# tum-vision/povar

Measured on AMD Instinct MI355X. Metric: power-series iterations/s (solve_pOSE terms per second), higher is better.
Workload: dtype f64

## Files before the change

### povar_amd/csrc/ck_layout.hpp

```cpp
#pragma once

#include <climits>
#include <cmath>
#include <cstring>

#include "lpl_layout.hpp"

namespace povar {

#ifndef POVAR_CK_HMAX_BUILD
#define POVAR_CK_HMAX_BUILD 16
#endif
constexpr int CK_HMAX = POVAR_CK_HMAX_BUILD;
constexpr int CK_LDS_BYTES = 160 * 1024;
constexpr int CK_FLAG_DUP = 1;
constexpr int CK_FLAG_COLD = 2;
constexpr uint32_t CK_NONE = 0xffffu;

constexpr double CK_UV_SCALE = 1e6, CK_UV_INV = 1e-6;
inline double ck_unpack_uv_host(int32_t k) {
  const double kd = (double)k;
  const double q0 = kd * CK_UV_INV;
  const double r = std::fma(-q0, CK_UV_SCALE, kd);
  return std::fma(r, CK_UV_INV, q0);
// ... 389 lines not shown
  K.n_part_rec = first[n_cams];
  K.part_range.assign(n_cams, make_int2(0, 0));
  for (int r0 = 0; r0 < n_cams; ++r0) K.part_range[cam_of_rank[r0]] = make_int2(first[r0], first[r0 + 1]);
  K.slot_rec.assign(L.wg_cams.size(), 0);
  {
    std::vector<int> next(first.begin(), first.end() - 1);
    for (int w = 0; w < grid; ++w)
      for (size_t a = 0; a < acc_rank_of[w].size(); ++a) K.slot_rec[(size_t)L.wg_cam_off[w] + a] = next[acc_rank_of[w][a]]++;
    std::vector<int> cold_rec((size_t)n_cold_chunks);
    for (int w = 0; w < grid; ++w)
      for (size_t i = 0; i < out[w].cold_rank.size(); ++i) cold_rec[(size_t)cold0_of[w] + i] = next[out[w].cold_rank[i]]++;
    K.uv.assign((size_t)(K.rows + CK_HMAX) * WAVE, make_double2(0, 0));
    K.src.assign((size_t)(K.rows + CK_HMAX) * WAVE, -1);
    if (shape.cold_q) K.cpos.assign((size_t)(K.rows + CK_HMAX) * WAVE, -1);
    K.li.assign((size_t)(K.li_rows + CK_HMAX) * WAVE, CK_NONE | (CK_NONE << 16));
    K.lane_cam.resize(K.tile.size() * WAVE);
    K.lane_acc.resize(K.tile.size() * WAVE);
    K.lane_seg.resize(K.tile.size() * WAVE);
    lpl_parallel(grid, n_threads, [&](int w) {
      const WgOut& o = out[w];
      std::copy(o.uv.begin(), o.uv.end(), K.uv.begin() + row0_of[w] * WAVE);
      std::copy(o.src.begin(), o.src.end(), K.src.begin() + row0_of[w] * WAVE);
      if (shape.cold_q) std::copy(o.cpos.begin(), o.cpos.end(), K.cpos.begin() + row0_of[w] * WAVE);
      std::copy(o.li.begin(), o.li.end(), K.li.begin() + li0_of[w] * WAVE);
      std::copy(o.lane_cam.begin(), o.lane_cam.end(), K.lane_cam.begin() + (size_t)tile0_of[w] * WAVE);
      std::copy(o.lane_seg.begin(), o.lane_seg.end(), K.lane_seg.begin() + (size_t)tile0_of[w] * WAVE);
      for (size_t i = 0; i < o.lane_acc.size(); ++i) {
        const int a = o.lane_acc[i];
        K.lane_acc[(size_t)tile0_of[w] * WAVE + i] = a >= 0 ? a : shape.cold_q ? -1 : ~cold_rec[(size_t)cold0_of[w] + (size_t)(~a)];
      }
    });
  }
  K.n_uv = K.uv.size();
  {
    const char* e = std::getenv("POVAR_CK_PACK");
    if (shape.need_uv && shape.slot_bytes == 48 && pack_uv && !(e && e[0] == '0')) ck_pack_uv(K, n_threads);
  }
  K.tick.assign(K.tile.size() * WAVE, 0);
  lpl_parallel(grid, n_threads, [&](int w) {
    std::vector<int> next((size_t)std::max(1, L.wg_cam_off[w + 1] - L.wg_cam_off[w]), 0);
    for (int b = 0; b < nb; ++b) {
      const int tb0 = K.bt_off[(size_t)w * nb + b], tb1 = K.bt_off[(size_t)w * nb + b + 1];
      for (int q0 = tb0; q0 < tb1; q0 += n_waves)
        for (int t = std::min(q0 + n_waves, tb1) - 1; t >= q0; --t)
          for (int lane = 0; lane < WAVE; ++lane) {
            const size_t i = (size_t)t * WAVE + lane;
            if (K.lane_cam[i] >= 0 && K.lane_acc[i] >= 0 && lane == ((K.lane_seg[i] >> 8) & 255))
              K.tick[i] = (uint16_t)next[K.lane_acc[i]]++;
          }
    }
  });
}

}
```

### povar_amd/csrc/povar_create.hip

```cpp
#include "povar_ctx.hpp"

std::mutex g_capture_mu;

int hot_acc_cap(int n_cams) {
  int cap = HOT_ACC_MAX;
  if (const char* e = std::getenv("POVAR_HOT_ACC")) cap = std::max(1, std::min(HOT_ACC_MAX, std::atoi(e)));
  return std::min(n_cams, cap);
}

struct Layout {
  std::vector<double2> uv, cm_uv;
  std::vector<int> cam, lm, meta, hot_cams, cam_hot, cc_slot, cc_lm, cc_item_off, cc_cam_item_off, long_lm, long_first, long_cnt, cm_slot, cm_lm, item_off,
      item_cam, cam_item_off, slot_of_obs, cold_pos;
  std::vector<int> c2_lm, c2_pos;
  std::vector<int2> c2_range;
  int n_bins = 0;
};

struct LayoutTmp {
  std::vector<int> seg_first, seg_last, rank;
  std::vector<char> is_long;
  std::vector<int64_t> cnt;
};

// ... 132 lines not shown
      L.c2_range.resize(n_cams);
      for (int c = 0; c < n_cams; ++c) {
        const int first = (int)L.c2_lm.size();
        const bool acc = rank[c] > 0 && rank[c] <= n_acc;
        if (!acc)
          for (int64_t p = cnt[c]; p < cnt[c + 1]; ++p) {
            L.c2_pos[L.cm_slot[p]] = (int)L.c2_lm.size();
            L.c2_lm.push_back(L.cm_lm[p]);
          }
        L.c2_range[c] = make_int2(first, (int)L.c2_lm.size());
      }
    }
  }
}

int ck_max_cams() {
  if (const char* e = std::getenv("POVAR_CK_MAX_CAMS")) return std::max(0, std::atoi(e));
  return 65535;
}

bool ck_upload(povar_ctx* c, povar_ctx::CkDev& D, const CkLayout& K, bool locked, size_t* bytes, bool need_uv) {
  bool ok = true;
  const bool usable = K.n_uv * sizeof(double2) < (1ull << 32) && c->n_cams <= ck_max_cams();
  D.ready = false;
  if (!usable) return true;
  auto guarded = [&](auto&& fn) {
    if (locked) {
      std::lock_guard<std::mutex> lk(g_capture_mu);
      fn();
    } else {
      fn();
    }
  };
  auto up = [&](auto& buf, const auto& v) {
    if (!ok) return;
    guarded([&] { ok = buf.alloc(std::max<size_t>(v.size(), 1), bytes) == hipSuccess; });
    const size_t piece = ((size_t)8 << 20) / sizeof(v[0]);
    for (size_t at = 0; ok && at < v.size() && !(locked && c->placer_cancel.load()); at += piece)
      guarded([&] {
        ok = hipMemcpy(buf.p + at, v.data() + at, std::min(piece, v.size() - at) * sizeof(v[0]), hipMemcpyHostToDevice) == hipSuccess;
      });
  };
  std::vector<int2> meta(K.lane_cam.size());
  for (size_t i = 0; i < meta.size(); ++i) {
    const int sg = K.lane_seg[i];
    meta[i] = make_int2(K.lane_cam[i] < 0 ? -1 : (K.lane_cam[i] | ((sg & 63) << 16) | (((sg >> 8) & 63) << 22)), K.lane_acc[i]);
  }
  D.packed = need_uv && K.packed;
  if (D.packed) up(D.uvp, K.uvp);
  else if (need_uv) up(D.uv, K.uv);
  up(D.li, K.li); up(D.src, K.src); up(D.tile, K.tile); up(D.lane_meta, meta);
  up(D.bt_off, K.bt_off); up(D.slot_rec, K.slot_rec); up(D.part_range, K.part_range);
  if (c->det_ck) { up(D.lcnt, K.lcnt_log2); up(D.tick, K.tick); }
  D.cold_q = K.cold_q;
  if (K.cold_q) up(D.cpos, K.cpos);
  if (ok) guarded([&] { ok = D.part.alloc((size_t)std::max(K.n_part_rec, 1) * 12, bytes) == hipSuccess; });
  if (ok && c->opt.robust_norm && !need_uv)
    guarded([&] { ok = D.w.alloc(std::max<size_t>(K.src.size(), 1), bytes) == hipSuccess; });
  D.nb = K.nb; D.slots = K.slots; D.n_part_rec = K.n_part_rec; D.max_acc = K.max_acc; D.max_tiles_bt = K.max_tiles_bt;
  D.stride = K.stride; D.n_capped_obs = K.n_capped_obs;
  D.rows = K.rows; D.li_rows = K.li_rows; D.n_chunks = K.n_chunks; D.n_cold_chunks = K.n_cold_chunks;
  D.w_lin_id = -1;
  D.ready = ok && !(locked && c->placer_cancel.load());
  if (!ok) D.release();
  return ok;
}

int res_upload(povar_ctx* c, const ResLayout& R) {
  povar_ctx::ResDev& D = c->res;
  int rc = 0;
  if ((rc = upload(D.lane_cam, R.lane_cam, c)) || (rc = upload(D.lane_seg, R.lane_seg, c)) ||
      (rc = upload(D.uv, R.uv, c)) || (rc = upload(D.lslot, R.lslot, c)) || (rc = upload(D.oslot, R.oslot, c)) ||
      (rc = upload(D.wave_h, R.wave_h, c)) || (rc = upload(D.lm_off, R.lm_off, c)) || (rc = upload(D.lm_id, R.lm_id, c)) ||
      (rc = upload(D.cam_off, R.cam_off, c)) || (rc = upload(D.cam_id, R.cam_id, c)) || (rc = upload(D.cam_zi, R.cam_zi, c)) ||
      (rc = upload(D.own_off, R.own_off, c)) || (rc = upload(D.own_cam, R.own_cam, c)) || (rc = upload(D.own_zi, R.own_zi, c)) ||
      (rc = upload(D.own_q, R.own_q, c)) || (rc = upload(D.oq_off, R.oq_off, c)) || (rc = upload(D.oq_rec, R.oq_rec, c)))
    return rc;
  const size_t n_part = (size_t)std::max(R.n_rec, 1) * 12, n_z = (size_t)c->n_cams * 12, n_nrm = (size_t)RES_MAX_WG * 2 * 2;
  if (n_part * sizeof(uint4) >= (1ull << 32)) return fail(-1, "resident series: partial records exceed a buffer descriptor");
  HIP_TRY(D.part.alloc(n_part, &c->bytes));
  HIP_TRY(D.zbuf.alloc(n_z, &c->bytes));
  HIP_TRY(D.nrm.alloc(n_nrm, &c->bytes));
  HIP_TRY(D.launch.alloc(4, &c->bytes));
  HIP_TRY(hipMemset(D.part.p, 0, n_part * sizeof(uint4)));
  HIP_TRY(hipMemset(D.zbuf.p, 0, n_z * sizeof(uint4)));
  HIP_TRY(hipMemset(D.nrm.p, 0, n_nrm * sizeof(uint4)));
  const unsigned one[4] = {1u, 0u, 0u, 0u};
  HIP_TRY(hipMemcpy(D.launch.p, one, sizeof(one), hipMemcpyHostToDevice));
  D.W = R.W; D.NW = R.NW; D.H = R.H; D.R = R.R; D.LS = R.LS; D.n_rec = R.n_rec; D.max_lm = R.max_lm; D.max_cam = R.max_cam;
  D.max_oq = R.max_oq; D.max_own = R.max_own; D.max_chunks = R.max_chunks; D.order = R.order; D.lds_bytes = R.lds_bytes;
  D.ready = true;
  return 0;
}

void res_build_for(int n_cams, int n_lms, const int32_t* lm_off, const int32_t* cam_idx, const double* obs,
                   const std::vector<int>& rank1, const std::vector<int>& slot_of_obs, int wgs, ResLayout& R) {
  build_res(n_cams, n_lms, lm_off, cam_idx, obs, rank1, slot_of_obs, wgs, 16, 1, 1, 2, 1, R);
  if (R.fits) return;
  build_res(n_cams, n_lms, lm_off, cam_idx, obs, rank1, slot_of_obs, wgs, 8, 2, 1, 4, 2, R);
}

int swap_in_placed_rows(povar_ctx* c, bool wait) {
  if (c->placement != 2) return 0;
  if (!wait && c->placer_state.load(std::memory_order_acquire) < 2) return 0;
  if (c->placer.joinable()) c->placer.join();
  if (c->placer_state.load(std::memory_order_acquire) != 2) {
// ... 780 lines not shown
```

### povar_amd/csrc/povar_ctx.hpp

```cpp
#pragma once
#include "../../include/povar_hip.h"

#include <hip/hip_runtime.h>
#include <rccl/rccl.h>

#include <algorithm>
#include <chrono>
#include <cmath>
#include <cstdio>
#include <cstdlib>
#include <cstring>
#include <memory>
#include <mutex>
#include <numeric>
#include <string>
#include <atomic>
#include <thread>
#include <vector>

#include "povar_kernels.hpp"
#include "povar_kernels_joint.hpp"
#include "povar_kernels_sc.hpp"
#include "povar_kernels_chol.hpp"
#include "lpl_layout.hpp"
// ... 57 lines not shown
  int64_t n_cold = 0;
  int n_cold_items = 0;
  povar_options opt{};
  hipStream_t stream = nullptr;
  size_t bytes = 0;
  int64_t lin_id = 0, views_lin_id = -1, aux_lin_id = -1;
  int64_t prep_id = 0, aux_prep_id = 0, prep_lin_id = -1;
  char* pin = nullptr;
  size_t pin_bytes = 0;

  std::vector<int> slot_of_obs;
  std::vector<int> lm_off;

  DevBuf<double2> uv, cm_uv, tiles;
  DevBuf<int2> cc_cam_range;
  DevBuf<int> cold_pos;
  DevBuf<int> c2_lm, c2_pos;
  DevBuf<int2> c2_range;
  DevBuf<double> c2_h;
  int64_t n_cold2 = 0;
  bool long_in_kernel = false;
  DevBuf<double2> v2_uv;
  DevBuf<int> v2_lm_of;
  DevBuf<int> v2_cw, v2_cpos, v2_lm_pos, v2_of_slot, v2_seg, v2_wg_tile_off, v2_wg_cam_off, v2_wg_cams, v2_wg_slot_rec, c3_lm;
  DevBuf<int2> v2_part_range, c3_range;
  DevBuf<int> c3_src, pl_c3_src;
  bool q_rows = false;
  DevBuf<double> c3_h, v2_part;
  int64_t n_cold3 = 0;
  int v2_max_slots = 0, v2_n_global = 0, v2_n_tail = 0, v2_strategy = 0;
  DevBuf<int4> v2_tile;
  DevBuf<double> v2_w, v2_lmrec;
  int64_t v2_rows = 0;
  std::thread placer;
  std::atomic<int> placer_state{0};
  std::atomic<bool> placer_cancel{false};
  DevBuf<double2> pl_uv;
  DevBuf<int> pl_cw, pl_cpos, pl_lm_pos, pl_lm_of, pl_of_slot;
  size_t pl_bytes = 0;
  int placement = 0;
  double placement_ms = 0;
  bool use_lpl = true;
  bool lpl_forced = false;
  bool use_lpl_prepare = true;
  struct CkDev {
    DevBuf<double2> uv;
    DevBuf<int2> uvp;
    bool packed = false;
    DevBuf<int> cpos;
    bool cold_q = false;
    DevBuf<uint32_t> li;
    DevBuf<int> src, bt_off, slot_rec;
    DevBuf<int2> lane_meta;
    DevBuf<int4> tile;
    DevBuf<int2> part_range;
    DevBuf<double> part, w;
    DevBuf<uint8_t> lcnt;
    DevBuf<uint16_t> tick;
    int nb = 0, slots = 0, n_part_rec = 0, max_acc = 0, max_tiles_bt = 0;
    int stride = 0;
    int64_t n_capped_obs = 0;
    int64_t rows = 0, li_rows = 0, n_chunks = 0, n_cold_chunks = 0;
    double build_ms = 0;
    int64_t w_lin_id = -1;
    bool ready = false;
    void release() {
      cpos.release(); cold_q = false;
      uv.release(); uvp.release(); li.release(); src.release(); lane_meta.release(); bt_off.release();
      slot_rec.release(); tile.release(); part_range.release(); part.release(); w.release();
      packed = false;
      lcnt.release(); tick.release();
      ready = false;
    }
  } ck, pl_ck,
    ckh, pl_ckh;
  struct ResDev {
    DevBuf<int> lane_cam, lane_seg, lslot, oslot, wave_h, lm_off, lm_id, cam_off, cam_id, cam_zi, own_off, own_cam, own_zi, oq_off, oq_rec;
    DevBuf<double2> uv;
    DevBuf<int2> own_q;
    DevBuf<uint4> part, zbuf, nrm;
    DevBuf<unsigned> launch;
    int W = 0, NW = 0, H = 0, R = 1, LS = 1, n_rec = 0, max_lm = 0, max_cam = 0, max_oq = 0, max_own = 0, max_chunks = 0, order = 0;
    size_t lds_bytes = 0;
    double build_ms = 0;
    bool ready = false;
    void release() {
      lane_cam.release(); lane_seg.release(); lslot.release(); oslot.release(); wave_h.release();
      lm_off.release(); lm_id.release(); cam_off.release(); cam_id.release(); cam_zi.release(); own_off.release(); own_cam.release();
      own_zi.release(); oq_off.release(); oq_rec.release();
      uv.release(); own_q.release(); part.release(); zbuf.release(); nrm.release(); launch.release();
      ready = false;
    }
  } res;
  int res_mode = -1;
  bool res_tuned = false, res_choice = false, res_failed = false;
  float res_tune_us[2] = {0, 0};
  bool res_check = false;
  int res_last_m = 0;
  double res_last_tol[2] = {0, 0};
  unsigned res_spin_limit = 1u << 18;
  bool deterministic = false;
  bool det_ck = false;
  bool det_check = false;
  bool fp32_terms = false;
  bool fp32_hold = false;
  int32_t fp32_last = 0;
  DevBuf<float2> ck32_uv;
  DevBuf<float> ck32_lmrec;
  DevBuf<float> ck32_pimg;
  DevBuf<int2> ck_zero_range;
  int ck_variant = 0;
  int ckh_variant = 0;
  bool ckh_tuned = false;
  float ckh_tune_us[2] = {0, 0};
  bool ck_auto = true;
  bool ck_tuned = false;
  bool ck_fresh[2] = {false, false};
  float ck_tune_us[2] = {0, 0};
  DevBuf<double4> q4c;
  DevBuf<int> lm_slot0, lm_cnt_dev;
  bool k1_qr = true;
// ... 211 lines not shown
```

### povar_amd/csrc/povar_kernels_ck.hpp

```cpp
#pragma once

#include "povar_kernels.hpp"

namespace povar {

constexpr int CK_ROWS = 16;

struct CkP {
  const double2* uv;
  const uint32_t* li;
  const double* w;
  const int4* tile;
  const int2* lane_meta;
  const int* bt_off;
  const int* slot_rec;
  int nb, slots;
  unsigned uv_bytes, li_bytes;
  const uint8_t* lcnt;
  const uint16_t* tick;
  int max_acc;
  int uv_packed;
  const int* cpos;
  double4* q4c;
};
__device__ inline double ck_unpack_uv(unsigned k) {
  const double kd = (double)(int)k;
  const double q0 = kd * 1e-6;
  const double r = __builtin_fma(-q0, 1e6, kd);
  return __builtin_fma(r, 1e-6, q0);
}
typedef unsigned __attribute__((ext_vector_type(4))) ck_u4;
constexpr int CK_ACC_STRIDE = 13;
__host__ __device__ inline size_t ck_lds_bytes_dev(int slots, int n_acc, int ng) { return 16 + (size_t)ng * slots * 48 + (size_t)n_acc * CK_ACC_STRIDE * 8 + 64; }

__device__ inline void ck_barrier() { asm volatile("s_waitcnt lgkmcnt(0)\n\ts_barrier" ::: "memory"); }

__device__ inline void ck_group_barrier(int* cnt, int& gen, int group_waves, int lane) {
  asm volatile("s_waitcnt lgkmcnt(0)" ::: "memory");
  gen += group_waves;
  if (lane == 0) __hip_atomic_fetch_add(cnt, 1, __ATOMIC_RELAXED, __HIP_MEMORY_SCOPE_WORKGROUP);
  while (__hip_atomic_load(cnt, __ATOMIC_RELAXED, __HIP_MEMORY_SCOPE_WORKGROUP) < gen) __builtin_amdgcn_s_sleep(2);
  asm volatile("" ::: "memory");
}

__host__ __device__ inline int ck_rank(int x) { return x < 0 ? -1 : (x & 0xffff); }
__host__ __device__ inline int ck_seg(int x) { return ((x >> 16) & 63) | (((x >> 22) & 63) << 8); }

__device__ inline void ck_forward_math(const LplObs& o, const double* zz, const double* P3, double hx, double hy, double hz,
                                       double* red) {
  const double d0 = hx * zz[0] + hy * zz[1] + hz * zz[2] + zz[3];
  const double d1 = hx * zz[4] + hy * zz[5] + hz * zz[6] + zz[7];
  const double d2 = hx * zz[8] + hy * zz[9] + hz * zz[10] + zz[11];
  const double a0 = o.w * (d0 - o.cu * d2);
  const double a1 = o.w * (d1 - o.cv * d2);
  const double a2 = o.w * (o.cuv * d2 - o.cu * d0 - o.cv * d1);
  red[0] = P3[0] * a0 + P3[3] * a1 + P3[6] * a2;
  red[1] = P3[1] * a0 + P3[4] * a1 + P3[7] * a2;
  red[2] = P3[2] * a0 + P3[5] * a1 + P3[8] * a2;
}

__device__ inline double ck_huber_w(const Dp& d, const double* P3, double hx, double hy, double hz, double2 uv) {
  const double p0 = P3[0] * hx + P3[1] * hy + P3[2] * hz + P3[9];
  const double p1 = P3[3] * hx + P3[4] * hy + P3[5] * hz + P3[10];
  const double p2 = P3[6] * hx + P3[7] * hy + P3[8] * hz + P3[11];
  const double a = p0 - uv.x * p2, b = p1 - uv.y * p2, c = p0 - uv.x, e = p1 - uv.y;
  const double r2 = d.sb * d.sb * (a * a + b * b) + d.sa * d.sa * (c * c + e * e);
  const double t = d.huber;
  double y = __builtin_amdgcn_rsq(r2);
  const double hr = 0.5 * r2;
  y = y * __builtin_fma(-hr * y, y, 1.5);
  y = y * __builtin_fma(-hr * y, y, 1.5);
  return r2 < t * t ? 1.0 : t * y;
}

__device__ inline void ck_obs_forward(const Dp& d, double2 uv, double w, const double* zz, const double* P3, double hx, double hy,
                                      double hz, double* lu, int S, uint32_t s) {
  LplObs o;
  o.set(d, uv, w);
  double red[3];
  ck_forward_math(o, zz, P3, hx, hy, hz, red);
  __hip_atomic_fetch_add(lu + s, red[0], __ATOMIC_RELAXED, __HIP_MEMORY_SCOPE_WORKGROUP);
  __hip_atomic_fetch_add(lu + s + 1, red[1], __ATOMIC_RELAXED, __HIP_MEMORY_SCOPE_WORKGROUP);
  __hip_atomic_fetch_add(lu + s + 2, red[2], __ATOMIC_RELAXED, __HIP_MEMORY_SCOPE_WORKGROUP);
}
__device__ inline void ck_obs_backward(const Dp& d, double2 uv, double w, const double* P3, double hx, double hy, double hz,
                                       const double* g, double* y) {
  LplObs o;
  o.set(d, uv, w);
  double q[3];
  lpl_backward(o, P3, g, q);
#pragma unroll
  for (int m = 0; m < 3; ++m) {
    y[4 * m] += hx * q[m];
    y[4 * m + 1] += hy * q[m];
    y[4 * m + 2] += hz * q[m];
    y[4 * m + 3] += q[m];
  }
}

struct CkRows {
  __amdgpu_buffer_rsrc_t uv, li, w;
};
__device__ inline CkRows ck_rows(const CkP& k) {
  CkRows R;
  R.uv = __builtin_amdgcn_make_buffer_rsrc(const_cast<double2*>(k.uv), 0, k.uv_bytes, 0x00020000);
  R.li = __builtin_amdgcn_make_buffer_rsrc(const_cast<uint32_t*>(k.li), 0, k.li_bytes, 0x00020000);
  R.w = __builtin_amdgcn_make_buffer_rsrc(const_cast<double*>(k.w), 0, k.w ? (k.uv_packed ? k.uv_bytes : k.uv_bytes / 2) : 0, 0x00020000);
  return R;
}
template <int D, bool ROBUST, bool PK = false>
struct CkStream {
  double2 uv[D];
  uint32_t w[D];
  __device__ inline void clear() {
#pragma unroll
    for (int i = 0; i < D; ++i) {
      uv[i] = make_double2(0, 0);
      w[i] = 0xffffffffu;
    }
  }
  __device__ inline void load(const CkRows& R, int row0, int li0, int j, int h, int lane, int i) {
    j = j < 0 ? 0 : (j >= h ? h - 1 : j);
    const unsigned ul = (unsigned)lane;
    const unsigned ro = (unsigned)(row0 + j) * (unsigned)(WAVE * 16), lo = (unsigned)(li0 + (j >> 1)) * (unsigned)(WAVE * 4);
    if (PK) {
      typedef unsigned __attribute__((ext_vector_type(2))) u2;
      const u2 a = __builtin_amdgcn_raw_buffer_load_b64(R.uv, ul * 8u, ro >> 1, 0);
      uv[i] = make_double2(ck_unpack_uv(a.x), ck_unpack_uv(a.y));
    } else {
      typedef unsigned __attribute__((ext_vector_type(4))) u4;
      const u4 a = __builtin_amdgcn_raw_buffer_load_b128(R.uv, ul * 16u, ro, 0);
      uv[i] = make_double2(__longlong_as_double(((long long)a.y << 32) | a.x), __longlong_as_double(((long long)a.w << 32) | a.z));
    }
    w[i] = __builtin_amdgcn_raw_buffer_load_b32(R.li, ul * 4u, lo, 0);
  }
  template <int DIR>
  __device__ inline void start(const CkRows& R, int row0, int li0, int h, int lane) {
#pragma unroll
    for (int i = 0; i < D; ++i) load(R, row0, li0, DIR > 0 ? i : h - 1 - i, h, lane, i);
  }
};
template <int D, bool ROBUST, bool PK>
__device__ inline void ck_forward_step(const Dp& d, const CkRows& k, CkStream<D, ROBUST, PK>& st, int row0, int li0, int h, int lane,
                                       const double* zz, const double* P3, const double* lh, double* lu, int S, int j, int i) {
  const double2 uv = st.uv[i];
  const uint32_t s = (st.w[i] >> (16 * (j & 1))) & 0xffffu;
  st.load(k, row0, li0, j + D, h, lane, i);
  if (s != 0xffffu) {
    const double hx = lh[s], hy = lh[s + 1], hz = lh[s + 2];
    const double rw = ROBUST ? ck_huber_w(d, P3, hx, hy, hz, uv) : 1.0;
    ck_obs_forward(d, uv, rw, zz, P3, hx, hy, hz, lu, S, s);
  }
}
template <int D, bool ROBUST, bool PK>
__device__ inline void ck_forward_rows(const Dp& d, const CkRows& k, CkStream<D, ROBUST, PK>& st, int row0, int li0, int h, int lane,
                                       const double* zz, const double* P3, const double* lh, double* lu, int S) {
  int n0 = 0;
#pragma nounroll
  for (; n0 + D <= h; n0 += D) {
#pragma unroll
    for (int i = 0; i < D; ++i) ck_forward_step<D, ROBUST, PK>(d, k, st, row0, li0, h, lane, zz, P3, lh, lu, S, n0 + i, i);
  }
#pragma unroll
  for (int i = 0; i < D - 1; ++i)
    if (n0 + i < h) ck_forward_step<D, ROBUST, PK>(d, k, st, row0, li0, h, lane, zz, P3, lh, lu, S, n0 + i, i);
}
template <int D, bool ROBUST, bool PK>
__device__ inline void ck_backward_step(const Dp& d, const CkRows& k, CkStream<D, ROBUST, PK>& st, int row0, int li0, int h, int lane,
                                        const double* P3, const double* lh, const double* lg, int S, double* y, int j, int i) {
  const double2 uv = st.uv[i];
  const uint32_t s = (st.w[i] >> (16 * (j & 1))) & 0xffffu;
  st.load(k, row0, li0, j - D, h, lane, i);
  if (s != 0xffffu) {
    const double hx = lh[s], hy = lh[s + 1], hz = lh[s + 2];
    const double rw = ROBUST ? ck_huber_w(d, P3, hx, hy, hz, uv) : 1.0;
    const double g[3] = {lg[s], lg[s + 1], lg[s + 2]};
    ck_obs_backward(d, uv, rw, P3, hx, hy, hz, g, y);
  }
}
template <int D, bool ROBUST, bool PK>
__device__ inline void ck_backward_rows(const Dp& d, const CkRows& k, CkStream<D, ROBUST, PK>& st, int row0, int li0, int h, int lane,
                                        const double* P3, const double* lh, const double* lg, int S, double* y) {
  int n0 = 0;
#pragma nounroll
  for (; n0 + D <= h; n0 += D) {
#pragma unroll
    for (int i = 0; i < D; ++i) ck_backward_step<D, ROBUST, PK>(d, k, st, row0, li0, h, lane, P3, lh, lg, S, y, h - 1 - (n0 + i), i);
  }
#pragma unroll
  for (int i = 0; i < D - 1; ++i)
    if (n0 + i < h) ck_backward_step<D, ROBUST, PK>(d, k, st, row0, li0, h, lane, P3, lh, lg, S, y, h - 1 - (n0 + i), i);
}

template <bool ROBUST, bool PK>
__device__ inline void ck_backward_rows_cold(const Dp& d, const CkP& k, const CkRows& R, int row0, int li0, int h, int lane,
                                             const double* P3, const double* lh, const double* lg, bool cold_lane, double* y) {
  for (int j = h - 1; j >= 0; --j) {
    CkStream<2, ROBUST, PK> one;
    one.load(R, row0, li0, j, h, lane, 0);
    const int cp = cold_lane ? k.cpos[(size_t)(row0 + j) * WAVE + lane] : -1;
    const double2 uv = one.uv[0];
    const uint32_t s = (one.w[0] >> (16 * (j & 1))) & 0xffffu;
    if (s != 0xffffu) {
      const double hx = lh[s], hy = lh[s + 1], hz = lh[s + 2];
      const double rw = ROBUST ? ck_huber_w(d, P3, hx, hy, hz, uv) : 1.0;
      const double g[3] = {lg[s], lg[s + 1], lg[s + 2]};
      LplObs o;
      o.set(d, uv, rw);
      double q[3];
      lpl_backward(o, P3, g, q);
      if (cp >= 0) {
        k.q4c[cp] = make_double4(q[0], q[1], q[2], 0.0);
      } else {
#pragma unroll
        for (int m = 0; m < 3; ++m) {
          y[4 * m] += hx * q[m];
          y[4 * m + 1] += hy * q[m];
          y[4 * m + 2] += hz * q[m];
          y[4 * m + 3] += q[m];
        }
      }
    }
  }
}

__device__ inline void ck_load_z(const Dp& d, int rank, double* zz) {
  const double2* r = reinterpret_cast<const double2*>(d.hot_rec + (size_t)rank * HOT_REC_STRIDE);
#pragma unroll
  for (int j = 0; j < 6; ++j) {
    const double2 v = r[j];
    zz[2 * j] = v.x;
    zz[2 * j + 1] = v.y;
  }
}
__device__ inline __amdgpu_buffer_rsrc_t ck_zimg_rsrc(const Dp& d) {
  return __builtin_amdgcn_make_buffer_rsrc(d.zimg, 0, (unsigned)d.n_cams * 96u, 0x00020000);
}
__device__ inline void ck_load_z_img(const Dp& d, int rank, double* zz) {
  const __amdgpu_buffer_rsrc_t ZR = ck_zimg_rsrc(d);
#pragma unroll
  for (int j = 0; j < 6; ++j) {
    const ck_u4 a = __builtin_amdgcn_raw_buffer_load_b128(ZR, (unsigned)rank * 96u + 16u * j, 0, 0);
    zz[2 * j] = __hiloint2double((int)a.y, (int)a.x);
    zz[2 * j + 1] = __hiloint2double((int)a.w, (int)a.z);
  }
}
__device__ inline void ck_load_p3(const Dp& d, int rank, double* P3) {
  const double2* r = reinterpret_cast<const double2*>(d.hot_rec + (size_t)rank * HOT_REC_STRIDE) + 6;
#pragma unroll
  for (int j = 0; j < 4; ++j) {
    const double2 v = r[j];
    P3[2 * j] = v.x;
    P3[2 * j + 1] = v.y;
  }
// ... 41 lines not shown
  }
}

template <int NW, int SD, bool DB, int NG, bool ROBUST, bool PK>
__global__ __launch_bounds__(NW * 64) void e0_ck(Dp d, CkP k, double* part_out) {
  const int done = d.flags[1];
  extern __shared__ double ck_lds[];
  constexpr int GW = NW / NG;
  const CkRows R = ck_rows(k);
  const int S = k.slots;
  const int lane0 = threadIdx.x & 63;
  const int wave_all = __builtin_amdgcn_readfirstlane((int)(threadIdx.x >> 6));
  const int grp = NG > 1 ? wave_all / GW : 0;
  const int wave = NG > 1 ? wave_all % GW : wave_all;
  int* gbase = reinterpret_cast<int*>(ck_lds);
  double* lh = ck_lds + 2 + (size_t)grp * 6 * S;
  double* lu = lh + 3 * S;
  double* acc = ck_lds + 2 + (size_t)NG * 6 * S;
  int* gcnt = gbase + grp;
  int ggen = 0;
  const V2& v = d.v2;
  const int cam0 = v.wg_cam_off[blockIdx.x];
  const int n_acc = v.wg_cam_off[blockIdx.x + 1] - cam0;
  const int t0 = __builtin_amdgcn_readfirstlane(v.wg_tile_off[blockIdx.x]);
  const int t1 = __builtin_amdgcn_readfirstlane(v.wg_tile_off[blockIdx.x + 1]);
  typedef const int __attribute__((address_space(4))) * cint_p;
  const cint_p tiles = (cint_p)(uintptr_t)k.tile;
  const cint_p bt = (cint_p)(uintptr_t)k.bt_off;
  if (done) return;
  auto group_barrier = [&]() {
    if (NG > 1) ck_group_barrier(gcnt, ggen, GW, lane0);
    else ck_barrier();
  };
  const int wave_t = (wave & ~3) | (((wave >> 2) & 1) ? 3 - (wave & 3) : (wave & 3));
  auto tile_of = [&](int tb0, int q) { return tb0 + q * GW + ((q & 1) ? GW - 1 - wave_t : wave_t); };
  constexpr int HM = 32 / NW > 0 ? 32 / NW : 1;
  double hn[HM][3];
  auto request_h = [&](int b, int lane) {
#pragma unroll
    for (int q = 0; q < HM; ++q) {
      hn[q][0] = hn[q][1] = hn[q][2] = 0;
      const int m = wave + q * GW;
      if (b < k.nb && t0 + b + k.nb * m < t1) {
        const double* rp = v.lmrec + ((size_t)(t0 + b + k.nb * m) * 9) * WAVE + lane;
        hn[q][0] = rp[0]; hn[q][1] = rp[WAVE]; hn[q][2] = rp[2 * WAVE];
      }
    }
  };
  int* lbt = reinterpret_cast<int*>(acc + (size_t)k.max_acc * CK_ACC_STRIDE);
  const bool bt_lds = k.nb + 1 <= 16;
  auto bt_of = [&](int i, bool first) {
    return (bt_lds && !first) ? __builtin_amdgcn_readfirstlane(lbt[i]) : bt[blockIdx.x * k.nb + i];
  };
  int rank_next = 0;
  auto request_first_meta = [&](int b, int lane) {
    rank_next = 0;
    if (b < k.nb) {
      const int tb0 = bt_of(b, b == grp), tb1 = bt_of(b + 1, b == grp);
      if (tb0 + wave_t < tb1) rank_next = ck_rank(k.lane_meta[(size_t)(tb0 + wave_t) * WAVE + lane].x);
    }
  };
  request_first_meta(grp, lane0);
  request_h(grp, lane0);
  for (int i = threadIdx.x; i < n_acc * CK_ACC_STRIDE; i += NW * 64) acc[i] = 0;
  if (NG > 1 && threadIdx.x < NG) gbase[threadIdx.x] = 0;
  if (bt_lds && (int)threadIdx.x <= k.nb) lbt[threadIdx.x] = k.bt_off[blockIdx.x * k.nb + threadIdx.x];
  if (NG > 1) ck_barrier();
  for (int b = grp; b < k.nb; b += NG) {
    int lane = lane0;
    asm volatile("" : "+v"(lane));
    const int tb0 = bt_of(b, b == grp), tb1 = bt_of(b + 1, b == grp);
    int q_t = 0;
    int t = tile_of(tb0, 0);
    int rank = rank_next;
    double zz[12] = {0, 0, 0, 0, 0, 0, 0, 0, 0, 0, 0, 0}, P3[12] = {0, 0, 0, 0, 0, 0, 0, 0, 0, 0, 0, 0};
    CkStream<SD, ROBUST, PK> st;
    st.clear();
    int row0 = 0, h = 0, fl = 0, li0 = 0;
    int tn = tile_of(tb0, 1);
    int rank_n = 0, rank_nn = 0;
    double zn[12] = {0, 0, 0, 0, 0, 0, 0, 0, 0, 0, 0, 0}, Pn[12] = {0, 0, 0, 0, 0, 0, 0, 0, 0, 0, 0, 0};
    CkStream<SD, ROBUST, PK> stn;
    stn.clear();
    int row0n = 0, hnx = 0, fln = 0, li0n = 0;
    if (t < tb1) {
      row0 = tiles[4 * t]; h = tiles[4 * t + 1]; fl = tiles[4 * t + 2]; li0 = tiles[4 * t + 3];
      if (tn < tb1) rank_n = ck_rank(k.lane_meta[(size_t)tn * WAVE + lane].x);
      ck_load_p<ROBUST>(d, rank < 0 ? 0 : rank, P3);
      st.template start<1>(R, row0, li0, h, lane);
    }
    if (t < tb1) ck_load_z_img(d, rank < 0 ? 0 : rank, zz);
#pragma unroll
    for (int q = 0; q < HM; ++q) {
      const int m = wave + q * GW;
      if (t0 + b + k.nb * m < t1) {
        const int s = m * WAVE + lane;
        lh[3 * s] = hn[q][0];
        lh[3 * s + 1] = hn[q][1];
        lh[3 * s + 2] = hn[q][2];
        lu[3 * s] = 0;
        lu[3 * s + 1] = 0;
        lu[3 * s + 2] = 0;
      }
    }
    for (int m = wave + HM * GW; t0 + b + k.nb * m < t1; m += GW) {
      const double* rp = v.lmrec + ((size_t)(t0 + b + k.nb * m) * 9) * WAVE + lane;
      const int s = m * WAVE + lane;
      lh[3 * s] = rp[0];
      lh[3 * s + 1] = rp[WAVE];
      lh[3 * s + 2] = rp[2 * WAVE];
      lu[3 * s] = 0;
      lu[3 * s + 1] = 0;
      lu[3 * s + 2] = 0;
    }
    auto request_next_fwd = [&]() {
      if (DB && tn < tb1) {
        const int tnn = tile_of(tb0, q_t + 2);
        row0n = tiles[4 * tn]; hnx = tiles[4 * tn + 1]; fln = tiles[4 * tn + 2]; li0n = tiles[4 * tn + 3];
        if (tnn < tb1) rank_nn = ck_rank(k.lane_meta[(size_t)tnn * WAVE + lane].x);
        const int rk = rank_n < 0 ? 0 : rank_n;
        ck_load_z_img(d, rk, zn);
        ck_load_p<ROBUST>(d, rk, Pn);
        stn.template start<1>(R, row0n, li0n, hnx, lane);
      }
    };
    request_next_fwd();
    group_barrier();
#pragma unroll
    for (int e = 0; e < 12; ++e) asm volatile("" : "+v"(zz[e]));
    while (t < tb1) {
      ck_forward_rows<SD, ROBUST, PK>(d, R, st, row0, li0, h, lane, zz, P3, lh, lu, S);
      if (tn >= tb1) break;
      t = tn;
      ++q_t;
      rank = rank_n;
      tn = tile_of(tb0, q_t + 1);
      if (DB) {
#pragma unroll
        for (int e = 0; e < 12; ++e) zz[e] = zn[e];
#pragma unroll
        for (int e = 0; e < (ROBUST ? 12 : 9); ++e) P3[e] = Pn[e];
        st = stn;
        row0 = row0n; h = hnx; fl = fln; li0 = li0n;
        rank_n = rank_nn;
        request_next_fwd();
      } else {
        row0 = tiles[4 * t]; h = tiles[4 * t + 1]; fl = tiles[4 * t + 2]; li0 = tiles[4 * t + 3];
        if (tn < tb1) rank_n = ck_rank(k.lane_meta[(size_t)tn * WAVE + lane].x);
        const int rk = rank < 0 ? 0 : rank;
        ck_load_z_img(d, rk, zz);
        ck_load_p<ROBUST>(d, rk, P3);
        st.template start<1>(R, row0, li0, h, lane);
      }
    }
    asm volatile("" : "+v"(lane));
    int acc_slot = 0, seg = 0;
    int tp = q_t > 0 ? tile_of(tb0, q_t - 1) : tb1;
    int rank_p = 0, acc_p = 0, seg_p = 0, rank_pp = 0, acc_pp = 0, seg_pp = 0;
    double G[HM][6];
#pragma unroll
    for (int q = 0; q < HM; ++q) {
#pragma unroll
      for (int e = 0; e < 6; ++e) G[q][e] = 0;
      const int m = wave + q * GW;
      if (t0 + b + k.nb * m < t1) {
        const double* rp = v.lmrec + ((size_t)(t0 + b + k.nb * m) * 9 + 3) * WAVE + lane;
#pragma unroll
        for (int e = 0; e < 6; ++e) G[q][e] = rp[e * WAVE];
      }
    }
    if (t < tb1) {
      const int2 me = k.lane_meta[(size_t)t * WAVE + lane];
      seg = ck_seg(me.x);
      acc_slot = me.y;
      if (tp < tb1) {
        const int2 mp = k.lane_meta[(size_t)tp * WAVE + lane];
        rank_p = ck_rank(mp.x);
        seg_p = ck_seg(mp.x);
        acc_p = mp.y;
      }
      st.template start<-1>(R, row0, li0, h, lane);
    }
    group_barrier();
    request_first_meta(b + NG, lane);
    request_h(b + NG, lane);
#pragma unroll
    for (int q = 0; q < HM; ++q) {
      const int m = wave + q * GW;
      if (t0 + b + k.nb * m < t1) {
        const int s = m * WAVE + lane;
        const double u0 = lu[3 * s], u1 = lu[3 * s + 1], u2 = lu[3 * s + 2];
        lu[3 * s] = G[q][0] * u0 + G[q][1] * u1 + G[q][2] * u2;
        lu[3 * s + 1] = G[q][1] * u0 + G[q][3] * u1 + G[q][4] * u2;
        lu[3 * s + 2] = G[q][2] * u0 + G[q][4] * u1 + G[q][5] * u2;
      }
    }
    for (int m = wave + HM * GW; t0 + b + k.nb * m < t1; m += GW) {
      const double* rp = v.lmrec + ((size_t)(t0 + b + k.nb * m) * 9 + 3) * WAVE + lane;
      const double g0 = rp[0], g1 = rp[WAVE], g2 = rp[2 * WAVE], g3 = rp[3 * WAVE], g4 = rp[4 * WAVE], g5 = rp[5 * WAVE];
      const int s = m * WAVE + lane;
      const double u0 = lu[3 * s], u1 = lu[3 * s + 1], u2 = lu[3 * s + 2];
      lu[3 * s] = g0 * u0 + g1 * u1 + g2 * u2;
      lu[3 * s + 1] = g1 * u0 + g3 * u1 + g4 * u2;
      lu[3 * s + 2] = g2 * u0 + g4 * u1 + g5 * u2;
    }
    auto request_next_bwd = [&]() {
      if (DB && tp < tb1) {
        const int tpp = q_t > 1 ? tile_of(tb0, q_t - 2) : tb1;
        row0n = tiles[4 * tp]; hnx = tiles[4 * tp + 1]; fln = tiles[4 * tp + 2]; li0n = tiles[4 * tp + 3];
        if (tpp < tb1) {
          const int2 mp = k.lane_meta[(size_t)tpp * WAVE + lane];
          rank_pp = ck_rank(mp.x);
          seg_pp = ck_seg(mp.x);
          acc_pp = mp.y;
        }
        ck_load_p<ROBUST>(d, rank_p < 0 ? 0 : rank_p, Pn);
        stn.template start<-1>(R, row0n, li0n, hnx, lane);
      }
    };
    request_next_bwd();
    group_barrier();
    while (t < tb1) {
      double y[12];
#pragma unroll
      for (int m = 0; m < 12; ++m) y[m] = 0;
      const bool cold_q = !ROBUST && k.cpos != nullptr && (fl & 2) != 0;
      if (cold_q) ck_backward_rows_cold<ROBUST, PK>(d, k, R, row0, li0, h, lane, P3, lh, lu, rank >= 0 && acc_slot < 0, y);
      else ck_backward_rows<SD, ROBUST, PK>(d, R, st, row0, li0, h, lane, P3, lh, lu, S, y);
      ck_flush_tile(y, fl, lane, rank, acc_slot, seg, acc, n_acc, cold_q ? nullptr : part_out);
      if (tp >= tb1) break;
      t = tp;
      --q_t;
      rank = rank_p; acc_slot = acc_p; seg = seg_p;
      tp = q_t > 0 ? tile_of(tb0, q_t - 1) : tb1;
      if (DB) {
#pragma unroll
        for (int e = 0; e < (ROBUST ? 12 : 9); ++e) P3[e] = Pn[e];
        st = stn;
        row0 = row0n; h = hnx; fl = fln; li0 = li0n;
        rank_p = rank_pp; acc_p = acc_pp; seg_p = seg_pp;
        request_next_bwd();
      } else {
        row0 = tiles[4 * t]; h = tiles[4 * t + 1]; fl = tiles[4 * t + 2]; li0 = tiles[4 * t + 3];
        if (tp < tb1) {
          const int2 mp = k.lane_meta[(size_t)tp * WAVE + lane];
          rank_p = ck_rank(mp.x);
          seg_p = ck_seg(mp.x);
          acc_p = mp.y;
        }
        ck_load_p<ROBUST>(d, rank < 0 ? 0 : rank, P3);
        st.template start<-1>(R, row0, li0, h, lane);
      }
    }
    group_barrier();
  }
  if (NG > 1) ck_barrier();
  const __amdgpu_buffer_rsrc_t PR = ck_part_rsrc(part_out);
  for (int i = threadIdx.x; i < n_acc * 6; i += NW * 64) {
    const int r = i / 6, m = 2 * (i % 6);
    const int rec = k.slot_rec[cam0 + r];
    ck_store_part(PR, (unsigned)rec * 96u + 16u * (unsigned)(i % 6), acc[r * CK_ACC_STRIDE + m], acc[r * CK_ACC_STRIDE + m + 1]);
  }
  if (d.p2p_epoch && blockIdx.x == 0 && threadIdx.x == 0) *d.p2p_epoch += 1;
}

POVAR_KERNEL __launch_bounds__(256) void ck_gather_w(const int* src, const double* w_lpl, double* w_ck, int64_t n) {
  const int64_t i = (int64_t)blockIdx.x * 256 + threadIdx.x;
  if (i >= n) return;
  const int s = src[i];
  w_ck[i] = s >= 0 ? w_lpl[s] : 0.0;
}

}
```

### povar_amd/csrc/povar_series.hip

```cpp
#include "povar_ctx.hpp"

CkP ck_params(const povar_ctx* c, const povar_ctx::CkDev& D) {
  return CkP{D.packed ? reinterpret_cast<const double2*>(D.uvp.p) : D.uv.p, D.li.p, D.w.p, D.tile.p, D.lane_meta.p, D.bt_off.p, D.slot_rec.p,
             D.nb, D.slots, (unsigned)(D.src.n * (D.packed ? sizeof(int2) : sizeof(double2))), (unsigned)(D.li.n * sizeof(uint32_t)),
             D.lcnt.p, D.tick.p, D.max_acc, D.packed ? 1 : 0, D.cold_q ? D.cpos.p : nullptr, c->q4c.p};
}

CkP ck_params(const povar_ctx* c) { return ck_params(c, c->ck); }


bool ck_det_possible(const povar_ctx* c) {
  return c->det_ck && c->ck.ready && c->ck.lcnt.p && c->ck.tick.p && c->use_lpl && c->opt.e0_mode == POVAR_E0_IMPLICIT &&
         c->ck.nb >= 1 && ck_lds_bytes_det(c->ck.slots, c->ck.max_acc) <= (size_t)CK_LDS_BYTES;
}

bool ck_det_active(const povar_ctx* c) { return ck_det_possible(c) && !c->joint; }

bool ck32_active(const povar_ctx* c) {
  return c->fp32_terms && !c->fp32_hold && !c->deterministic && !c->joint && c->ck.ready && c->use_lpl && c->opt.e0_mode == POVAR_E0_IMPLICIT_LDSACC &&
         c->ck32_lmrec.p && c->ck32_pimg.p && (c->ck.packed || c->ck32_uv.p) &&
         ck32_lds_bytes(c->ck.slots, c->ck.max_acc) <= (size_t)CK_LDS_BYTES;
}

bool ck_active(const povar_ctx* c) {
  if (c->fp32_terms && !c->fp32_hold) return ck32_active(c);
  if (c->deterministic) return ck_det_active(c);
  return c->ck_variant > 0 && c->ck.ready && c->use_lpl && !c->joint && c->opt.e0_mode == POVAR_E0_IMPLICIT_LDSACC &&
         ck_variant_fits(c, c->ck_variant);
}

bool ckh_det_possible(const povar_ctx* c) {
  return c->det_ck && c->ckh.ready && c->ckh.lcnt.p && c->ckh.tick.p && c->use_lpl && c->opt.e0_mode == POVAR_E0_IMPLICIT &&
         c->ckh.stride == CKH_STRIDE && c->ckh.slots <= CKH_STRIDE && ckh_lds_bytes_det(c->ckh.max_acc) <= (size_t)CK_LDS_BYTES;
}

bool ckh_active(const povar_ctx* c) {
  if (c->deterministic) return c->joint && ckh_det_possible(c);
  return c->joint && c->ckh_variant > 0 && c->ckh.ready && c->use_lpl && c->opt.e0_mode == POVAR_E0_IMPLICIT_LDSACC &&
         (c->ckh.stride == CKH_STRIDE || c->ckh.stride == CKH_STRIDE_WIDE) && c->ckh.slots <= c->ckh.stride &&
         ckh_lds_bytes(c->ckh.max_acc, c->ckh.stride) <= (size_t)CK_LDS_BYTES;
}

void ck_dp(const povar_ctx* c, Dp& da) {
  const povar_ctx::CkDev& D = c->joint ? c->ckh : c->ck;
  da.hot_part = D.part.p;
  da.part_range = D.part_range.p;
  da.cmv.src = nullptr;
  da.q_rows = 0;
  if (D.cold_q) return;
  da.cmv.cam_range = c->ck_zero_range.p;
  da.cmv.n = 0;
}

template <int NW, int SD, bool DB, int NG>
void launch_e0_ck_t(povar_ctx* c, const Dp& da) {
  const CkP k = ck_params(c);
  const size_t lds = ck_lds_bytes(c->ck.slots, c->ck.max_acc, NG);
  const bool huber = c->opt.robust_norm == POVAR_NORM_HUBER;
// ... 904 lines not shown
```

Before: 18710.

## Prefetch first-tile headers and ranks early via precomputed per-block tables

Adds host-built per-plane tables holding the first tile header and camera ranks for each wave's first tile. The kernel uses them at entry, and at the end of each bin it issues the next bin's first-tile loads, so first-tile setup is hoisted out of the dependent load chain at the start of each bin. It also stores packed uv words raw in the stream and unpacks them at use rather than at load. The cost is extra device tables, more live registers and a shape static_assert that limits which GW/NG configurations may use the early path.

```diff
diff --git a/povar_amd/csrc/ck_layout.hpp b/povar_amd/csrc/ck_layout.hpp
--- a/povar_amd/csrc/ck_layout.hpp
+++ b/povar_amd/csrc/ck_layout.hpp
@@ -465,4 +465,29 @@
   });
 }
 
-}
+constexpr int CK_FIRST_PLANES = 4;
+inline int ck_first_gw(int plane) { return plane == 0 ? 16 : plane == 1 ? 12 : 8; }
+inline int ck_first_ng(int plane) { return plane == 3 ? 2 : 1; }
+inline void ck_first_tables(const CkLayout& K, int grid, std::vector<int2>& meta, std::vector<int4>& hdr) {
+  meta.assign((size_t)CK_FIRST_PLANES * grid * 16 * WAVE, make_int2(0xffff | (0xffff << 16), -1));
+  hdr.assign((size_t)CK_FIRST_PLANES * grid * 16, make_int4(0, 0, 0, 0));
+  const int nb = K.nb;
+  auto rank16 = [&](int t, int lane) { const int r = K.lane_cam[(size_t)t * WAVE + lane]; return r < 0 ? 0xffff : (r & 0xffff); };
+  for (int p = 0; p < CK_FIRST_PLANES; ++p) {
+    const int gw = ck_first_gw(p), ng = ck_first_ng(p);
+    for (int w = 0; w < grid; ++w)
+      for (int s = 0; s < ng * gw; ++s) {
+        const int b = s / gw, j = s % gw;
+        if (b >= nb) continue;
+        const int tb0 = K.bt_off[(size_t)w * nb + b], tb1 = K.bt_off[(size_t)w * nb + b + 1];
+        const int t = tb0 + j, t2 = tb0 + gw + (gw - 1 - j);
+        if (t >= tb1) continue;
+        const size_t at = ((size_t)p * grid + w) * 16 + s;
+        hdr[at] = K.tile[t];
+        for (int lane = 0; lane < WAVE; ++lane)
+          meta[at * WAVE + lane] = make_int2(rank16(t, lane) | ((t2 < tb1 ? rank16(t2, lane) : 0xffff) << 16), t);
+      }
+  }
+}
+
+}
diff --git a/povar_amd/csrc/povar_create.hip b/povar_amd/csrc/povar_create.hip
--- a/povar_amd/csrc/povar_create.hip
+++ b/povar_amd/csrc/povar_create.hip
@@ -208,6 +208,12 @@
   up(D.li, K.li); up(D.src, K.src); up(D.tile, K.tile); up(D.lane_meta, meta);
   up(D.bt_off, K.bt_off); up(D.slot_rec, K.slot_rec); up(D.part_range, K.part_range);
   if (c->det_ck) { up(D.lcnt, K.lcnt_log2); up(D.tick, K.tick); }
+  if (need_uv) {
+    std::vector<int2> fm;
+    std::vector<int4> fh;
+    ck_first_tables(K, K.nb > 0 ? (int)((K.bt_off.size() - 1) / K.nb) : 0, fm, fh);
+    up(D.first_meta, fm); up(D.first_hdr, fh);
+  }
   D.cold_q = K.cold_q;
   if (K.cold_q) up(D.cpos, K.cpos);
   if (ok) guarded([&] { ok = D.part.alloc((size_t)std::max(K.n_part_rec, 1) * 12, bytes) == hipSuccess; });
diff --git a/povar_amd/csrc/povar_ctx.hpp b/povar_amd/csrc/povar_ctx.hpp
--- a/povar_amd/csrc/povar_ctx.hpp
+++ b/povar_amd/csrc/povar_ctx.hpp
@@ -133,6 +133,8 @@
     DevBuf<uint32_t> li;
     DevBuf<int> src, bt_off, slot_rec;
     DevBuf<int2> lane_meta;
+    DevBuf<int2> first_meta;
+    DevBuf<int4> first_hdr;
     DevBuf<int4> tile;
     DevBuf<int2> part_range;
     DevBuf<double> part, w;
@@ -147,7 +149,7 @@
     bool ready = false;
     void release() {
       cpos.release(); cold_q = false;
-      uv.release(); uvp.release(); li.release(); src.release(); lane_meta.release(); bt_off.release();
+      uv.release(); uvp.release(); li.release(); src.release(); lane_meta.release(); bt_off.release(); first_meta.release(); first_hdr.release();
       slot_rec.release(); tile.release(); part_range.release(); part.release(); w.release();
       packed = false;
       lcnt.release(); tick.release();
diff --git a/povar_amd/csrc/povar_kernels_ck.hpp b/povar_amd/csrc/povar_kernels_ck.hpp
--- a/povar_amd/csrc/povar_kernels_ck.hpp
+++ b/povar_amd/csrc/povar_kernels_ck.hpp
@@ -22,6 +22,8 @@
   int uv_packed;
   const int* cpos;
   double4* q4c;
+  const int2* first_meta;
+  const int4* first_hdr;
 };
 __device__ inline double ck_unpack_uv(unsigned k) {
   const double kd = (double)(int)k;
@@ -111,14 +113,17 @@
 template <int D, bool ROBUST, bool PK = false>
 struct CkStream {
   double2 uv[D];
+  unsigned pk[D][2];
   uint32_t w[D];
   __device__ inline void clear() {
 #pragma unroll
     for (int i = 0; i < D; ++i) {
       uv[i] = make_double2(0, 0);
+      pk[i][0] = pk[i][1] = 0;
       w[i] = 0xffffffffu;
     }
   }
+  __device__ inline double2 get(int i) const { return PK ? make_double2(ck_unpack_uv(pk[i][0]), ck_unpack_uv(pk[i][1])) : uv[i]; }
   __device__ inline void load(const CkRows& R, int row0, int li0, int j, int h, int lane, int i) {
     j = j < 0 ? 0 : (j >= h ? h - 1 : j);
     const unsigned ul = (unsigned)lane;
@@ -126,7 +131,8 @@
     if (PK) {
       typedef unsigned __attribute__((ext_vector_type(2))) u2;
       const u2 a = __builtin_amdgcn_raw_buffer_load_b64(R.uv, ul * 8u, ro >> 1, 0);
-      uv[i] = make_double2(ck_unpack_uv(a.x), ck_unpack_uv(a.y));
+      pk[i][0] = a.x;
+      pk[i][1] = a.y;
     } else {
       typedef unsigned __attribute__((ext_vector_type(4))) u4;
       const u4 a = __builtin_amdgcn_raw_buffer_load_b128(R.uv, ul * 16u, ro, 0);
@@ -143,7 +149,7 @@
 template <int D, bool ROBUST, bool PK>
 __device__ inline void ck_forward_step(const Dp& d, const CkRows& k, CkStream<D, ROBUST, PK>& st, int row0, int li0, int h, int lane,
                                        const double* zz, const double* P3, const double* lh, double* lu, int S, int j, int i) {
-  const double2 uv = st.uv[i];
+  const double2 uv = st.get(i);
   const uint32_t s = (st.w[i] >> (16 * (j & 1))) & 0xffffu;
   st.load(k, row0, li0, j + D, h, lane, i);
   if (s != 0xffffu) {
@@ -168,7 +174,7 @@
 template <int D, bool ROBUST, bool PK>
 __device__ inline void ck_backward_step(const Dp& d, const CkRows& k, CkStream<D, ROBUST, PK>& st, int row0, int li0, int h, int lane,
                                         const double* P3, const double* lh, const double* lg, int S, double* y, int j, int i) {
-  const double2 uv = st.uv[i];
+  const double2 uv = st.get(i);
   const uint32_t s = (st.w[i] >> (16 * (j & 1))) & 0xffffu;
   st.load(k, row0, li0, j - D, h, lane, i);
   if (s != 0xffffu) {
@@ -199,7 +205,7 @@
     CkStream<2, ROBUST, PK> one;
     one.load(R, row0, li0, j, h, lane, 0);
     const int cp = cold_lane ? k.cpos[(size_t)(row0 + j) * WAVE + lane] : -1;
-    const double2 uv = one.uv[0];
+    const double2 uv = one.get(0);
     const uint32_t s = (one.w[0] >> (16 * (j & 1))) & 0xffffu;
     if (s != 0xffffu) {
       const double hx = lh[s], hy = lh[s + 1], hz = lh[s + 2];
@@ -347,44 +353,95 @@
   auto bt_of = [&](int i, bool first) {
     return (bt_lds && !first) ? __builtin_amdgcn_readfirstlane(lbt[i]) : bt[blockIdx.x * k.nb + i];
   };
-  int rank_next = 0;
-  auto request_first_meta = [&](int b, int lane) {
-    rank_next = 0;
+  constexpr bool EARLY = !ROBUST && SD == 2;
+  int tb0_next = 0, tb1_next = 0, rank_next = 0, rank_next2 = 0;
+  ck_u4 hdr_next = {0, 0, 0, 0};
+  auto request_first_meta = [&](int b, int lane, bool ranks) {
+    tb0_next = tb1_next = 0;
     if (b < k.nb) {
-      const int tb0 = bt_of(b, b == grp), tb1 = bt_of(b + 1, b == grp);
-      if (tb0 + wave_t < tb1) rank_next = ck_rank(k.lane_meta[(size_t)(tb0 + wave_t) * WAVE + lane].x);
+      tb0_next = bt_of(b, b == grp);
+      tb1_next = bt_of(b + 1, b == grp);
+    }
+    if (!ranks) return;
+    rank_next = rank_next2 = 0;
+    hdr_next = ck_u4{0, 0, 0, 0};
+    if (b < k.nb) {
+      const int tf = tile_of(tb0_next, 0), tf2 = tile_of(tb0_next, 1);
+      if (tf < tb1_next && !EARLY) rank_next = ck_rank(k.lane_meta[(size_t)tf * WAVE + lane].x);
+      if (tf < tb1_next && EARLY) {
+        const __amdgpu_buffer_rsrc_t TR = __builtin_amdgcn_make_buffer_rsrc(const_cast<int4*>(k.tile), 0, 0x7ffffff0, 0x00020000);
+        hdr_next = __builtin_amdgcn_raw_buffer_load_b128(TR, 0u, (unsigned)tf * 16u, 0);
+        rank_next = ck_rank(k.lane_meta[(size_t)tf * WAVE + lane].x);
+        if (tf2 < tb1_next) rank_next2 = ck_rank(k.lane_meta[(size_t)tf2 * WAVE + lane].x);
+      }
     }
   };
-  request_first_meta(grp, lane0);
-  request_h(grp, lane0);
+  double zz[12] = {0, 0, 0, 0, 0, 0, 0, 0, 0, 0, 0, 0}, P3[12] = {0, 0, 0, 0, 0, 0, 0, 0, 0, 0, 0, 0};
+  CkStream<SD, ROBUST, PK> st;
+  st.clear();
+  int row0 = 0, h = 0, fl = 0, li0 = 0;
+  auto request_first_tile = [&](int lane, bool have) {
+    const int tf = tile_of(tb0_next, 0);
+    const int rk = rank_next < 0 ? 0 : rank_next;
+    if (have && EARLY) {
+      row0 = __builtin_amdgcn_readfirstlane((int)hdr_next.x);
+      h = __builtin_amdgcn_readfirstlane((int)hdr_next.y);
+      fl = __builtin_amdgcn_readfirstlane((int)hdr_next.z);
+      li0 = __builtin_amdgcn_readfirstlane((int)hdr_next.w);
+      ck_load_z_img(d, rk, zz);
+      ck_load_p<ROBUST>(d, rk, P3);
+      st.template start<1>(R, row0, li0, h, lane);
+    } else if (have) {
+      const int tf2 = tile_of(tb0_next, 1);
+      row0 = tiles[4 * tf]; h = tiles[4 * tf + 1]; fl = tiles[4 * tf + 2]; li0 = tiles[4 * tf + 3];
+      if (tf2 < tb1_next) rank_next2 = ck_rank(k.lane_meta[(size_t)tf2 * WAVE + lane].x);
+      ck_load_p<ROBUST>(d, rk, P3);
+      st.template start<1>(R, row0, li0, h, lane);
+      ck_load_z_img(d, rk, zz);
+    } else {
+#pragma unroll
+      for (int e = 0; e < 12; ++e) zz[e] = P3[e] = 0;
+      st.clear();
+      row0 = h = fl = li0 = 0;
+    }
+  };
+  int bt_first = 0;
+  if (bt_lds && (int)threadIdx.x <= k.nb) bt_first = k.bt_off[blockIdx.x * k.nb + threadIdx.x];
+  if (EARLY) {
+    static_assert(!EARLY || (NG == 1 && (GW == 16 || GW == 12 || GW == 8)) || (NG == 2 && GW == 8), "shape without a first-request table");
+    constexpr int PLANE = NG > 1 ? 3 : GW == 16 ? 0 : GW == 12 ? 1 : 2;
+    const unsigned fs = (PLANE * gridDim.x + blockIdx.x) * 16u + (unsigned)(grp * GW + wave_t);
+    const int2 fm = k.first_meta[(size_t)fs * WAVE + lane0];
+    const __amdgpu_buffer_rsrc_t HR = __builtin_amdgcn_make_buffer_rsrc(const_cast<int4*>(k.first_hdr), 0, 0x7ffffff0, 0x00020000);
+    hdr_next = __builtin_amdgcn_raw_buffer_load_b128(HR, 0u, fs * 16u, 0);
+    request_h(grp, lane0);
+    const int r1 = fm.x & 0xffff, r2 = (fm.x >> 16) & 0xffff;
+    rank_next = r1 == 0xffff ? -1 : r1;
+    rank_next2 = r2 == 0xffff ? -1 : r2;
+    request_first_tile(lane0, __builtin_amdgcn_readfirstlane(fm.y) >= 0);
+    request_first_meta(grp, lane0, false);
+  } else {
+    request_first_meta(grp, lane0, true);
+    request_h(grp, lane0);
+  }
   for (int i = threadIdx.x; i < n_acc * CK_ACC_STRIDE; i += NW * 64) acc[i] = 0;
   if (NG > 1 && threadIdx.x < NG) gbase[threadIdx.x] = 0;
-  if (bt_lds && (int)threadIdx.x <= k.nb) lbt[threadIdx.x] = k.bt_off[blockIdx.x * k.nb + threadIdx.x];
+  if (bt_lds && (int)threadIdx.x <= k.nb) lbt[threadIdx.x] = bt_first;
   if (NG > 1) ck_barrier();
   for (int b = grp; b < k.nb; b += NG) {
     int lane = lane0;
     asm volatile("" : "+v"(lane));
-    const int tb0 = bt_of(b, b == grp), tb1 = bt_of(b + 1, b == grp);
+    const int tb0 = tb0_next, tb1 = tb1_next;
     int q_t = 0;
     int t = tile_of(tb0, 0);
     int rank = rank_next;
-    double zz[12] = {0, 0, 0, 0, 0, 0, 0, 0, 0, 0, 0, 0}, P3[12] = {0, 0, 0, 0, 0, 0, 0, 0, 0, 0, 0, 0};
-    CkStream<SD, ROBUST, PK> st;
-    st.clear();
-    int row0 = 0, h = 0, fl = 0, li0 = 0;
     int tn = tile_of(tb0, 1);
-    int rank_n = 0, rank_nn = 0;
+    if (!EARLY) request_first_tile(lane, t < tb1);
+    int rank_n = rank_next2, rank_nn = 0;
     double zn[12] = {0, 0, 0, 0, 0, 0, 0, 0, 0, 0, 0, 0}, Pn[12] = {0, 0, 0, 0, 0, 0, 0, 0, 0, 0, 0, 0};
     CkStream<SD, ROBUST, PK> stn;
     stn.clear();
     int row0n = 0, hnx = 0, fln = 0, li0n = 0;
-    if (t < tb1) {
-      row0 = tiles[4 * t]; h = tiles[4 * t + 1]; fl = tiles[4 * t + 2]; li0 = tiles[4 * t + 3];
-      if (tn < tb1) rank_n = ck_rank(k.lane_meta[(size_t)tn * WAVE + lane].x);
-      ck_load_p<ROBUST>(d, rank < 0 ? 0 : rank, P3);
-      st.template start<1>(R, row0, li0, h, lane);
-    }
-    if (t < tb1) ck_load_z_img(d, rank < 0 ? 0 : rank, zz);
 #pragma unroll
     for (int q = 0; q < HM; ++q) {
       const int m = wave + q * GW;
@@ -477,7 +534,7 @@
       st.template start<-1>(R, row0, li0, h, lane);
     }
     group_barrier();
-    request_first_meta(b + NG, lane);
+    request_first_meta(b + NG, lane, true);
     request_h(b + NG, lane);
 #pragma unroll
     for (int q = 0; q < HM; ++q) {
@@ -547,6 +604,7 @@
         st.template start<-1>(R, row0, li0, h, lane);
       }
     }
+    if (EARLY) request_first_tile(lane, tile_of(tb0_next, 0) < tb1_next);
     group_barrier();
   }
   if (NG > 1) ck_barrier();
diff --git a/povar_amd/csrc/povar_series.hip b/povar_amd/csrc/povar_series.hip
--- a/povar_amd/csrc/povar_series.hip
+++ b/povar_amd/csrc/povar_series.hip
@@ -3,7 +3,8 @@
 CkP ck_params(const povar_ctx* c, const povar_ctx::CkDev& D) {
   return CkP{D.packed ? reinterpret_cast<const double2*>(D.uvp.p) : D.uv.p, D.li.p, D.w.p, D.tile.p, D.lane_meta.p, D.bt_off.p, D.slot_rec.p,
              D.nb, D.slots, (unsigned)(D.src.n * (D.packed ? sizeof(int2) : sizeof(double2))), (unsigned)(D.li.n * sizeof(uint32_t)),
-             D.lcnt.p, D.tick.p, D.max_acc, D.packed ? 1 : 0, D.cold_q ? D.cpos.p : nullptr, c->q4c.p};
+             D.lcnt.p, D.tick.p, D.max_acc, D.packed ? 1 : 0, D.cold_q ? D.cpos.p : nullptr, c->q4c.p,
+             D.first_meta.p, D.first_hdr.p};
 }
 
 CkP ck_params(const povar_ctx* c) { return ck_params(c, c->ck); }
```

Result: faster. 19400, median of 6 (+3.7%).
